# nitishsaDire/objectDetection_ssd

Hardware: AMD Instinct MI355X
Metric: images/sec SSD300-VGG16 train step (higher is better)
Workload: dtype f32 (tensors, accumulators, loss, SGD; the Winograd-domain products of the layers with >= 256 reduction channels are formed from three EXACT bf16 limbs per f32 operand on the bf16 MFMA -- six limb products per f32 product, dropped terms <= 2^-26 -- measured no further from f64 than the f32 MFMA; SSD

## Files before the change

### include/ssd_gfx950.h

```cpp
#ifndef SSD_GFX950_H
#define SSD_GFX950_H

#include <stddef.h>
#include <stdint.h>

#ifdef __cplusplus
extern "C" {
#endif

#define SSD_ABI_VERSION 1

enum ssd_status {
    SSD_OK = 0,
    SSD_ERR_BAD_SHAPE = -1,
    SSD_ERR_WORKSPACE = -2,
    SSD_ERR_NULL = -3,
    SSD_ERR_LAUNCH = -4,
    SSD_ERR_ALIGN = -5
};

int ssd_abi_version(void);
const char* ssd_status_string(int status);

typedef struct ssd_conv_geom {
// ... 100 lines not shown
int ssd_wino4_dy_transform(const float* dy, int ldy, const ssd_conv_geom* g, float* wgrad_planes, float* dgrad_planes_out,
                           float* bias_partial, void* stream);
size_t ssd_wino4_wgrad_gemm_workspace(const ssd_conv_geom* g, int ldy);
int ssd_wino4_wgrad_gemm(const float* wgrad_planes, const float* x_planes, int ldy, const float* bias_partial, float* dw_oihw, float* dbias,
                         const ssd_conv_geom* g, void* workspace, size_t workspace_bytes, void* stream);
int ssd_wino4_dy_transform_pooled(const float* dpool, const unsigned char* argmax, const float* y_pooled, int Hp, int Wp, int ldy,
                                  const ssd_conv_geom* g, float* wgrad_planes, float* dgrad_planes_out, float* bias_partial, void* stream);
int ssd_conv3x3_wino_wgrad_planes_pooled(const float* planes, const float* dpool, const unsigned char* argmax, const float* y_pooled,
                                         int Hp, int Wp, int ldy, float* dw_oihw, float* dbias, const ssd_conv_geom* g,
                                         float* dgrad_planes_out, void* workspace, size_t workspace_bytes, void* stream);
int ssd_conv3x3_wino_fwd_keep_bits(const float* x, const float* U_fwd, const float* bias, float* y, int ldy, const ssd_conv_geom* g, int relu,
                                   float* planes_keep, uint64_t* relu_bits_out, void* workspace, size_t workspace_bytes, void* stream);
int ssd_conv3x3_wino_fwd_pool_bits(const float* x, const float* U_fwd, const float* bias, float* y_pooled, uint8_t* argmax,
                                   const ssd_conv_geom* g, int ceil_mode, float* planes_keep, uint64_t* relu_bits_out, void* workspace,
                                   size_t workspace_bytes, void* stream);
int ssd_conv3x3_wino_dgrad_bits(const float* dy, int ldy, const float* U_bwd, int Co_pad, float* dx, const uint64_t* relu_bits, int accumulate,
                                const ssd_conv_geom* g, void* workspace, size_t workspace_bytes, void* stream);
int ssd_conv3x3_wino_dgrad_planes_bits(const float* dy_planes, const float* U_bwd, int Co_pad, float* dx, const uint64_t* relu_bits,
                                       int accumulate, const ssd_conv_geom* g, void* workspace, size_t workspace_bytes, void* stream);
int ssd_conv3x3_wino_wgrad_planes(const float* planes, const float* dy, int ldy, float* dw_oihw, float* dbias, const ssd_conv_geom* g,
                                  float* dgrad_planes_out, void* workspace, size_t workspace_bytes, void* stream);
int ssd_conv3x3_wino_dgrad_planes(const float* dy_planes, const float* U_bwd, int Co_pad, float* dx, const float* relu_mask,
                                  int accumulate, const ssd_conv_geom* g, void* workspace, size_t workspace_bytes, void* stream);
int ssd_conv1_first_wino_fwd(const float* x_nchw, const float* w_rows, const float* bias, float* planes, uint64_t* relu_bits, int N, int H, int W,
                             void* stream);
int ssd_conv3x3_wino_fwd_from_planes(const float* planes, const float* U_fwd, const float* bias, float* y, int ldy, float* y_pooled, uint8_t* argmax,
                                     const ssd_conv_geom* g, int relu, int ceil_mode, void* workspace, size_t workspace_bytes, void* stream);
int ssd_wino_weights_adj(const float* w_oihw, float* U_adj, int Co, int Ci, int Co_pad, void* stream);
size_t ssd_wino4_adj_planes_floats(const ssd_conv_geom* g);
int ssd_conv3x3_wino_dgrad_adj_gemm(const float* y_planes, int ldy, const float* U_adj, float* md_planes, const ssd_conv_geom* g, void* stream);
int ssd_wino4_adj_output(const float* md_planes, float* dx, const float* relu_mask, const uint64_t* relu_bits, int accumulate,
                         const ssd_conv_geom* g, void* stream);
int ssd_wino4_adj_output_to_planes(const float* md_planes, const float* relu_mask, const uint64_t* relu_bits, const ssd_conv_geom* g,
                                   const ssd_conv_geom* g_below, float* y_planes, float* bias_partial, void* stream);
int ssd_tune_set_wino_bias_tail(int on);
int ssd_tune_set_wino_xform_blocks(int blocks);
int ssd_tune_set_wino_fused(int mode);
int ssd_gemm_planes_x3v2(const void* a3, const void* w3, float* out, int M, int K, int N, int n_rows, int nbatch, int dither, void* stream);
int ssd_tune_set_x3_big(int mode);
int ssd_tune_set_x3_mfma(int rows);
int ssd_tune_set_gemm_nt(int mode);
int ssd_wino_uses_x3(int mo, int K);
int ssd_tune_set_wino_x3(int on);
size_t ssd_gemm_x3_weights_bytes(int rows, int K, int nbatch);
int ssd_gemm_x3_split_weights(const float* w, void* w3, int rows, int K, int nbatch, void* stream);
int ssd_gemm_planes_x3(const float* a, const void* w3, float* out, int M, int K, int N, int n_rows, int nbatch, void* stream);
// ... 158 lines not shown
```

### objectdetection_ssd_amd/Model.py

```python
from __future__ import annotations

import numbers
from typing import Dict, List, Optional

import torch
import torch.nn as nn

from . import ops
from .Util import ANCHORS_PER_CELL, ANCHORS_PER_CELL_512, subsampling

N_CLASSES = 21
MAX_FOREGROUND = 255
_VGG_CFG = (64, 64, "M", 128, 128, "M", 256, 256, 256, "M", 512, 512, 512, "M", 512, 512, 512, "M")


class _VGG16(nn.Module):

    def __init__(self):
        super().__init__()
        layers: List[nn.Module] = []
        cin = 3
        for v in _VGG_CFG:
            if v == "M":
                layers.append(nn.MaxPool2d(kernel_size=2, stride=2))
# ... 65 lines not shown
    for op in op_list:
        if op["op"] in ("conv", "conv_first"):
            names += [op["p"] + ".weight", op["p"] + ".bias"]
        elif op["op"] == "l2norm":
            names.append(op["p"])
        elif op["op"] == "head":
            names += [op["p"] + "_bb.weight", op["p"] + "_bb.bias", op["p"] + "_cl.weight", op["p"] + "_cl.bias"]
    return names


def _cat_flat(a: torch.Tensor, b: torch.Tensor) -> torch.Tensor:
    if (a.dim() == 1 and b.dim() == 1 and a.is_contiguous() and b.is_contiguous() and a.dtype == b.dtype
            and a.untyped_storage().data_ptr() == b.untyped_storage().data_ptr() and a.storage_offset() + a.numel() == b.storage_offset()):
        return torch.as_strided(a, (a.numel() + b.numel(),), (1,), a.storage_offset())
    return torch.cat((a, b))


class _Elided:

    dtype = torch.float32

    def __init__(self, shape):
        self.shape = tuple(shape)


class _SinkDict(dict):

    def __init__(self, sink):
        super().__init__()
        self._sink = sink
        self._held = None

    def __setitem__(self, name, tensor):
        super().__setitem__(name, tensor)
        if self._held is not None:
            self._held.append((name, tensor))
        else:
            self._sink(name, tensor)

    def hold(self):
        if self._held is None:
            self._held = []

    def release(self):
        held, self._held = self._held or [], None
        for name, tensor in held:
# ... 28 lines not shown
        self.pool_after: Dict[str, dict] = {}
        for op in self.ops:
            readers = [o for o in self.ops if o["x"] == op["y"]] if op["op"] == "conv" else []
            if (len(readers) == 1 and readers[0]["op"] == "pool" and (readers[0]["k"], readers[0]["s"], readers[0]["pad"]) == (2, 2, 0)
                    and op["relu"] and op["co"] % 4 == 0):
                self.pool_after[op["y"]] = readers[0]
        self._conv_of = {o["y"]: o for o in self.ops if o["op"] == "conv"}
        self.grad_sink = None
        self.grad_out = None
        self.sink_owns_grads = False
        self.sink_early = False
        self._test_side_delay = None
        self.grad_tap = None
        self.dual_dy = True
        self.keep_planes = True
        self.fuse_pool = True
        self.lazy_pool_grad = True
        self.first_fused = True
        self.wino_dilated = True
        self.relu_bits = True
        self.adjoint_dgrad = True
        self.first_wino = False
        self.adjoint_chain = True
        self.prof = None
        self.bf16 = False
        self.bf16_tensors = True
        self.x3 = False
        self.wino = True

    def _timed(self, label, tag, flops, fn):
        if self.prof is None:
            return fn()
        executed = flops
        if isinstance(flops, tuple):
            flops, executed = flops
        e0, e1 = torch.cuda.Event(enable_timing=True), torch.cuda.Event(enable_timing=True)
        e0.record()
        out = fn()
        e1.record()
        self.prof.append((label, tag, flops, e0, e1, executed))
        return out

    def schedule_key(self) -> tuple:
        return (self.bf16, self.bf16_tensors, self.x3, self.wino, self.WINO_TILE, self.WINO_MIN_CI, self.WINO_MIN_HW,
                self.WINO_WGRAD_MAX_HW, self.WINO_WGRAD_MIN_CI, self.X31_MIN_PIXELS, ops.wino_x3(4, 256), self.adjoint_dgrad,
                self.adjoint_chain, self.keep_planes, self.dual_dy, self.fuse_pool, self.lazy_pool_grad, self.relu_bits, self.wino_dilated,
                self.first_fused, self.first_wino, self.overlap_wgrad, self.batch_weights)

    def uses_weight_table(self) -> bool:
        return self.batch_weights and not self.x3 and (not self.bf16 or self.bf16_tensors)

    def _layouts(self, key: str, tensors, co_pad: int, need_bwd: bool):
        sig = tuple((t.data_ptr(), t._version) for t in tensors)
        ent = self._wcache.get(key)
        if ent is None or ent[0] != sig:
            w = tensors[0] if len(tensors) == 1 else torch.cat(list(tensors), 0)
            ent = [sig, w.detach().contiguous(), None, None]
            ent[2] = ops.weight_ohwi(ent[1], co_pad)
            self._wcache[key] = ent
        if need_bwd and ent[3] is None:
            ent[3] = ops.weight_ihwo(ent[1], co_pad)
        if self.x3 or (self.bf16 and not self.bf16_tensors):
            if len(ent) == 4:
                ent += [None, None]
            if ent[4] is None:
                ent[4] = ops.weight_split3(ent[2])
            if need_bwd and ent[5] is None:
                ent[5] = ops.weight_split3(ent[3])
            if self.x3:
                return ent[4], ent[5]
# ... 616 lines not shown
                                                         db_out=self._gout(name + ".bias")))
                        if side_ctx[0] is not None and defer:
                            deferred.append(wg)
                        else:
                            wg()
                        dw = None
                    if dw is not None:
                        grads[op["p"] + ".weight"], grads[op["p"] + ".bias"] = dw, db
                if self._wino_ok(g):
                    _, ub = self._wino_weights(op["p"], (P[op["p"] + ".weight"],), op["co"], adj=self._adj_ok(g))
                    if self._adj_ok(g):
                        raise RuntimeError(f"{op['p']}: its filter planes are laid out for the adjoint data gradient, which needs the forward's kept planes "
                                           "(the engine's keep_planes / dual_dy / adjoint_dgrad switches must not change between a forward and its backward)")
                    bits = aux.pop("bits:" + op["p"], None) if (dyp is not None or ops.wino_uses_full(g, 1) or isinstance(T[op["x"]], _Elided)) else None
                    def dgrad_rot(dx, acc, mask, dy=dy, ub=ub, g=g, dyp=dyp, bits=bits, name=op["p"]):
                        if isinstance(mask, _Elided):
                            if bits is None:
                                raise RuntimeError(f"{name}: its input was not stored and no ReLU bits were kept for its data gradient")
                            mask_t = None
                        else:
                            mask_t = mask
                        return ops.conv2d_dgrad_wino(None if isinstance(dy, ops.PooledGrad) else dy, ub, g, dx, mask_t, acc, planes=dyp,
                                                     bits=bits if mask is not None else None)
                    deliver(op["x"], lambda dx, acc, mask: self._timed("dgrad " + op["p"], "winograd_3x3", ops.wino_flops(g),
                                                                       lambda: dgrad_rot(dx, acc, mask)))
                    continue
                if self._x31_ok(g) and not to_bf16:
                    _, w3b = self._x31_weights(op["p"], (P[op["p"] + ".weight"],), op["co"])
                    deliver(op["x"], lambda dx, acc, mask: self._timed(
                        "dgrad " + op["p"], "gemm_planes_x3_kernel (1x1)", ops.conv_flops(g),
                        lambda: ops.conv1x1_dgrad_x3(dy, w3b, g, dx, mask, acc)))
                    continue
                _, wb = self._layouts(op["p"], (P[op["p"] + ".weight"],), op["co"], True)
                if to_bf16:
                    def boundary(dx, acc, mask, dy=dy, wb=wb, g=g, name=op["p"]):
                        if acc or mask is not None or dx is not None:
                            raise RuntimeError("the bf16 trunk's boundary tensor must have one consumer and no ReLU of its own")
                        d32 = self._timed("dgrad " + name, ops.igemm_tile(g, 1, self.bf16, self.x3) if self.prof is not None else "", ops.conv_flops(g),
                                          lambda: ops.conv2d_dgrad(dy, wb, g, None, None, False, bf16=self.bf16, w3=self._planes(name, True)))
                        return ops.cast_bf16(d32)
                    deliver(op["x"], boundary)
                    continue
                deliver(op["x"], lambda dx, acc, mask: self._timed(
                    "dgrad " + op["p"], ops.igemm_tile(g, 1, self.bf16, self.x3) if self.prof is not None else "", ops.conv_flops(g),
                    lambda: ops.conv2d_dgrad_x3(dy, wb, g, dx, mask, acc) if self.x3 else
                    ops.conv2d_dgrad(dy, wb, g, dx, mask, acc, bf16=self.bf16, w3=self._planes(op["p"], True))))
# ... 4 lines not shown
                yout = T[op["y"]]
                deliver(op["x"], lambda dx, acc, mask: (
                    ops.PooledGrad(dy, am, yout, xin.shape)
                    if (self.lazy_pool_grad and isinstance(xin, _Elided) and mask is not None and not acc and dx is None
                        and (op["k"], op["s"], op["pad"]) == (2, 2, 0)) else
                    ops.maxpool_bwd(dy, am, tuple(xin.shape), op["k"], op["s"], op["pad"], dx, y_gate=yout)
                    if (mask is not None and not acc) else
                    ops.maxpool_bwd(dy, am, tuple(xin.shape), op["k"], op["s"], op["pad"], dx, mask, acc)))
            elif kind == "l2norm":
                dy = G.pop(op["y"])
                xin = T[op["x"]]
                gamma = P[op["p"]].detach().reshape(-1)
                box = {}

                def run(dx, acc, mask, xin=xin, gamma=gamma, dy=dy, box=box):
                    if acc or mask is not None:
                        raise RuntimeError("L2-norm backward must deliver the first, non-final gradient of its input")
                    dx, box["dg"] = ops.l2norm_bwd(xin, gamma, dy, dg_out=self._gout(op["p"]))
                    return dx
                deliver(op["x"], run)
                grads[op["p"]] = box["dg"].reshape(P[op["p"]].shape)
            elif kind == "conv_first":
                dy = G.pop(op["y"])
                if need[op["p"] + ".weight"] or need[op["p"] + ".bias"]:
                    g = aux[op["y"]]
                    col = T["x_col"]
                    if col is None:
                        dw, db = self._timed("wgrad " + op["p"], "conv_first_wgrad_kernel", 2.0 * dy.numel() * 27,
                                             lambda: (ops.conv1_first_wgrad_bf16 if dy.dtype == torch.bfloat16 else ops.conv1_first_wgrad)(T["x"], dy, True))
                    else:
                        dw, db = self._timed("wgrad " + op["p"], ops.wgrad_tile(g, self.bf16) if self.prof is not None else "", 2.0 * dy.numel() * 27,
                                             lambda: ops.conv2d_wgrad(col, dy, g, g.Co, True))
                    grads[op["p"] + ".weight"], grads[op["p"] + ".bias"] = ops.first_weight_grad(dw), db
        if not joined:
            main.wait_event(join_event)
        if side_done is not None:
            main.wait_event(side_done)
        if wgrad_used:
            main.wait_event(self._wgrad_stream.record_event())
        if held:
            grads.release()
        return grads


class _SSD300Function(torch.autograd.Function):
    @staticmethod
# ... 171 lines not shown
```

### objectdetection_ssd_amd/_lib.py

```python
from __future__ import annotations

import ctypes as C
import os

PKG = os.path.dirname(os.path.abspath(__file__))
LIB_PATH = os.path.join(PKG, "libssd_gfx950.so")

SSD_ABI_VERSION = 1


class ConvGeom(C.Structure):
    _fields_ = [(n, C.c_int32) for n in ("N", "H", "W", "Ci", "Ho", "Wo", "Co", "R", "S", "stride", "pad", "dil")]


class ImageDesc(C.Structure):
    _fields_ = [("src_offset", C.c_int64)] + [(n, C.c_int32) for n in (
        "src_h", "src_w", "canvas_h", "canvas_w", "place_top", "place_left", "crop_top", "crop_left", "crop_h", "crop_w",
        "flip", "reserved")]


class WeightJob(C.Structure):
    _fields_ = [("w0", C.c_void_p), ("w1", C.c_void_p), ("out_fwd", C.c_void_p), ("out_bwd", C.c_void_p)] + [(n, C.c_int32) for n in (
        "co0", "co", "ci", "taps", "co_pad", "kind", "pad0", "pad1")]

# ... 96 lines not shown
    "ssd_conv3x3_wino_fwd": (_I, [_P, _P, _P, _P, _I, _G, _I, _I, _P, _Z, _P]),
    "ssd_conv3x3_wino_fwd_pool": (_I, [_P, _P, _P, _P, _P, _G, _I, _P, _P, _Z, _P]),
    "ssd_conv3x3_wino_fwd_keep": (_I, [_P, _P, _P, _P, _I, _G, _I, _P, _P, _Z, _P]),
    "ssd_weight_job_blocks": (_I, [_P]),
    "ssd_weights_prepare": (_I, [_P, _P, _I, _I, _P]),
    "ssd_wino4_bias_partial_floats": (_Z, [_G, _I]),
    "ssd_wino4_dy_transform": (_I, [_P, _I, _G, _P, _P, _P, _P]),
    "ssd_wino_weights_adj": (_I, [_P, _P, _I, _I, _I, _P]),
    "ssd_conv1_first_wino_fwd": (_I, [_P, _P, _P, _P, _P, _I, _I, _I, _P]),
    "ssd_conv3x3_wino_fwd_from_planes": (_I, [_P, _P, _P, _P, _I, _P, _P, _G, _I, _I, _P, _Z, _P]),
    "ssd_wino4_adj_planes_floats": (_Z, [_G]),
    "ssd_conv3x3_wino_dgrad_adj_gemm": (_I, [_P, _I, _P, _P, _G, _P]),
    "ssd_wino4_adj_output": (_I, [_P, _P, _P, _P, _I, _G, _P]),
    "ssd_wino4_adj_output_to_planes": (_I, [_P, _P, _P, _G, _G, _P, _P, _P]),
    "ssd_wino4_dy_transform_pooled": (_I, [_P, _P, _P, _I, _I, _I, _G, _P, _P, _P, _P]),
    "ssd_conv3x3_wino_wgrad_planes_pooled": (_I, [_P, _P, _P, _P, _I, _I, _I, _P, _P, _G, _P, _P, _Z, _P]),
    "ssd_wino4_wgrad_gemm_workspace": (_Z, [_G, _I]),
    "ssd_wino4_wgrad_gemm": (_I, [_P, _P, _I, _P, _P, _P, _G, _P, _Z, _P]),
    "ssd_conv3x3_wino_fwd_keep_bits": (_I, [_P, _P, _P, _P, _I, _G, _I, _P, _P, _P, _Z, _P]),
    "ssd_conv3x3_wino_fwd_pool_bits": (_I, [_P, _P, _P, _P, _P, _G, _I, _P, _P, _P, _Z, _P]),
    "ssd_conv3x3_wino_dgrad_planes_bits": (_I, [_P, _P, _I, _P, _P, _I, _G, _P, _Z, _P]),
    "ssd_conv3x3_wino_wgrad_planes": (_I, [_P, _P, _I, _P, _P, _G, _P, _P, _Z, _P]),
    "ssd_conv3x3_wino_dgrad_planes": (_I, [_P, _P, _I, _P, _P, _I, _G, _P, _Z, _P]),
    "ssd_conv3x3_wino_dgrad": (_I, [_P, _I, _P, _I, _P, _P, _I, _G, _I, _P, _Z, _P]),
    "ssd_conv3x3_wino_wgrad_workspace": (_Z, [_G, _I, _I]),
    "ssd_conv3x3_wino_wgrad": (_I, [_P, _P, _I, _P, _P, _G, _I, _P, _Z, _P]),
    "ssd_tune_set_wino_wgrad_tn": (_I, [_I]),
    "ssd_tune_set_wino_fused": (_I, [_I]),
    "ssd_tune_set_gemm_nt": (_I, [_I]),
    "ssd_tune_set_wino_bias_tail": (_I, [_I]),
    "ssd_tune_set_batched_units": (_I, [_I]),
    "ssd_tune_set_dgrad_parity": (_I, [_I]),
    "ssd_tune_set_wino_full": (_I, [_I]),
    "ssd_conv3x3_wino_uses_full": (_I, [_G, _I]),
    "ssd_conv3x3_wino_dgrad_bits": (_I, [_P, _I, _P, _I, _P, _P, _I, _G, _P, _Z, _P]),
    "ssd_tune_set_wino_xform_blocks": (_I, [_I]),
    "ssd_tune_set_wino_fused_stamps": (_I, [_P]),
    "ssd_tune_set_wino_fused_stagger": (_I, [_I]),
    "ssd_prof_gemm_begin": (_I, []),
    "ssd_prof_gemm_collect": (_I, [_P, _P, _I]),
    "ssd_prof_gemm_collect_kinds": (_I, [_P, _P, _P, _I]),
    "ssd_tune_set_igemm": (_I, [_I, _I]),
    "ssd_tune_set_igemm_lds_pad": (_I, [_I]),
    "ssd_tune_set_igemm_stamps": (_I, [_P]),
    "ssd_tune_set_wgrad": (_I, [_I, _I, _I]),
    "ssd_tune_set_wgrad_patch": (_I, [_I]),
# ... 57 lines not shown
```

### objectdetection_ssd_amd/csrc/wino_fused.hip

```cpp
#include "common.h"

namespace {

__device__ constexpr float F4_AT[4][6] = {{1, 1, 1, 1, 1, 0}, {0, 1, -1, 2, -2, 0}, {0, 1, 1, 4, 4, 0}, {0, 1, -1, 8, -8, 1}};

struct FusedParams {
    const float* V;
    const float* U;
    size_t plane_v, plane_u;
    int tiles, K, Nrows, Nout;
    int groups, nblk_n;
    float* out; int ldo; int Cvalid;
    const float* bias; const float* mask; const unsigned long long* mask_bits; int relu, accumulate;
    int H, W, TH, TW;
    float* yp; uint8_t* am; int Ho, Wo;
    unsigned long long* stamps;
    int stagger;
};

constexpr int FG = 32, FN = 64, FK = 64;
#ifndef WF_NS
#define WF_NS 5
#define WF_PD 3
#endif
constexpr int NS = WF_NS, PD = WF_PD;
constexpr int STAGE_F = (FG + FN) * FK;
constexpr int LOADS = 3;
constexpr int YS_F = FG * 16 * FN;
constexpr int LDS_F = NS * STAGE_F > YS_F ? NS * STAGE_F : YS_F;
static_assert(NS - PD >= 2, "a slot is re-filled no earlier than two barriers after its last read");
static_assert(LDS_F * 4 <= 160 * 1024, "LDS");

typedef __attribute__((address_space(3))) void lds_void;

template <int N> __device__ __forceinline__ void wait_vmcnt() { asm volatile("s_waitcnt vmcnt(%0)" ::"n"(N) : "memory"); }

template <int KCN>
__global__ __launch_bounds__(512, 2) void wino4_gemm_out_kernel(const FusedParams p) {
    __shared__ __attribute__((aligned(16))) float lds[LDS_F];
    const int tid = threadIdx.x, lane = tid & 63;
    const int wave = __builtin_amdgcn_readfirstlane(tid >> 6);
    const int mb = wave >> 2, nbw = wave & 3;
    const int nblk = p.groups * p.nblk_n;
    const int lid = xcd_swizzle(blockIdx.x, nblk);
    const int grp = lid / p.nblk_n, nb = lid - grp * p.nblk_n;
    const int tile0 = grp * FG, n0 = nb * FN;
    constexpr int S = 36 * KCN;
    const bool stamp = p.stamps != nullptr && (blockIdx.x & 15) == 0 && tid == 0;
    unsigned long long ts[8] = {0, 0, 0, 0, 0, 0, 0, 0};
    if (stamp) ts[0] = __builtin_readcyclecounter();
    if (p.stagger > 0 && blockIdx.x < 256) {
        const long long want = (long long)((blockIdx.x >> 3) & 7) * p.stagger;
        const long long t0 = (long long)__builtin_readcyclecounter();
        while ((long long)__builtin_readcyclecounter() - t0 < want) __builtin_amdgcn_s_sleep(64);
    }

    const int lrow = lane >> 4, pc = lane & 15;
    unsigned src_off[LOADS];
    bool is_a[LOADS];
    int lds_off[LOADS];
#pragma unroll
    for (int i = 0; i < LOADS; ++i) {
// ... 64 lines not shown
#endif
        __builtin_amdgcn_sched_barrier(0);
        mma4(c, cur, 1);
        mma4(c, cur, 2);
        __builtin_amdgcn_sched_barrier(0);
        if (s + 1 < S) {
            const int issued = (s + PD + 1 < S ? s + PD + 1 : S);
            const int ahead = issued - s - 2;
            if (ahead >= 3) wait_vmcnt<3 * LOADS>();
            else if (ahead == 2) wait_vmcnt<2 * LOADS>();
            else if (ahead == 1) wait_vmcnt<LOADS>();
            else wait_vmcnt<0>();
            __builtin_amdgcn_s_barrier();
            asm volatile("" ::: "memory");
            load_frags(nxt, (s + 1) % NS);
        }
        __builtin_amdgcn_sched_barrier(0);
        mma4(c, cur, 3);
    }

    if (stamp) ts[2] = __builtin_readcyclecounter();
    float* ys = lds;
    const int C4 = p.Nout >> 2;
    __builtin_amdgcn_s_barrier();
#pragma unroll
    for (int r = 0; r < 4; ++r) {
        float t[4][6];
#pragma unroll
        for (int b = 0; b < 6; ++b) {
            const float m0 = acc[b][r], m1 = acc[6 + b][r], m2 = acc[12 + b][r], m3 = acc[18 + b][r], m4 = acc[24 + b][r], m5 = acc[30 + b][r];
            const float s1 = m1 + m2, d1 = m1 - m2, s2 = m3 + m4, d2 = m3 - m4;
            t[0][b] = m0 + s1 + s2;
            t[1][b] = d1 + 2.f * d2;
            t[2][b] = s1 + 4.f * s2;
            t[3][b] = d1 + 8.f * d2 + m5;
        }
        float* dst = ys + (size_t)((mb * 16 + 4 * kq + r) * 16) * FN + nbw * 16 + r15;
#pragma unroll
        for (int i = 0; i < 4; ++i) {
            const float s1 = t[i][1] + t[i][2], d1 = t[i][1] - t[i][2], s2 = t[i][3] + t[i][4], d2 = t[i][3] - t[i][4];
            dst[(i * 4 + 0) * FN] = t[i][0] + s1 + s2;
            dst[(i * 4 + 1) * FN] = d1 + 2.f * d2;
            dst[(i * 4 + 2) * FN] = s1 + 4.f * s2;
            dst[(i * 4 + 3) * FN] = d1 + 8.f * d2 + t[i][5];
        }
    }
    asm volatile("s_waitcnt lgkmcnt(0)" ::: "memory");
    __builtin_amdgcn_s_barrier();
    if (stamp) ts[3] = __builtin_readcyclecounter();
    {
        const int tl = tid >> 4, c4l = tid & 15;
        const int tile = tile0 + tl, c4 = (n0 >> 2) + c4l;
        if (tile < p.tiles && c4 < C4) {
            const int tw = tile % p.TW, th = (tile / p.TW) % p.TH, n = tile / (p.TW * p.TH);
            const float* src = ys + (size_t)(tl * 16) * FN + c4l * 4;
            f32x4 bv = {0.f, 0.f, 0.f, 0.f};
            if (p.bias != nullptr) {
#pragma unroll
                for (int e = 0; e < 4; ++e) bv[e] = c4 * 4 + e < p.Cvalid ? p.bias[c4 * 4 + e] : 0.f;
            }
            if (p.yp == nullptr) {
                const unsigned long long word = p.mask_bits != nullptr ? p.mask_bits[(size_t)tile * C4 + c4] : 0ull;
#pragma unroll
                for (int a = 0; a < 4; ++a) {
                    const int oh = 4 * th + a;
                    if (oh >= p.H) continue;
#pragma unroll
                    for (int b = 0; b < 4; ++b) {
                        const int ow = 4 * tw + b;
                        if (ow >= p.W) continue;
                        f32x4 v = *reinterpret_cast<const f32x4*>(src + (a * 4 + b) * FN) + bv;
                        const size_t idx = (((size_t)n * p.H + oh) * p.W + ow) * p.ldo + c4 * 4;
                        if (p.accumulate) v += *reinterpret_cast<const f32x4*>(p.out + idx);
// ... 74 lines not shown
    return SSD_OK;
}
extern "C" int ssd_tune_set_wino_fused_stamps(uint64_t* device_buffer) {
    g_fused_stamps = reinterpret_cast<unsigned long long*>(device_buffer);
    return SSD_OK;
}

__attribute__((visibility("hidden"))) int ssd_internal_wino4_gemm_out(const float* V, const float* U, int tiles, int K, int Nrows, int Nout,
                                                                       float* out, int ldo, int Cvalid, const float* bias, const float* mask,
                                                                       const unsigned long long* mask_bits, int relu, int accumulate, int H, int W,
                                                                       int TH, int TW, float* yp, uint8_t* am, int Ho, int Wo, hipStream_t st) {
    if ((K != 64 && K != 128 && K != 256) || tiles <= 0 || Nout <= 0 || Nout % 4 != 0 || Nrows <= 0) return SSD_ERR_BAD_SHAPE;
    if ((size_t)tiles * K >= (1ull << 32) || (size_t)Nrows * K >= (1ull << 32)) return SSD_ERR_BAD_SHAPE;
    FusedParams p;
    p.V = V; p.U = U;
    p.plane_v = (size_t)tiles * K; p.plane_u = (size_t)Nrows * K;
    p.tiles = tiles; p.K = K; p.Nrows = Nrows; p.Nout = Nout;
    p.groups = ssd_cdiv(tiles, FG); p.nblk_n = ssd_cdiv(Nout, FN);
    p.out = out; p.ldo = ldo; p.Cvalid = Cvalid; p.bias = bias; p.mask = mask; p.mask_bits = mask_bits; p.relu = relu; p.accumulate = accumulate;
    p.H = H; p.W = W; p.TH = TH; p.TW = TW;
    p.yp = yp; p.am = am; p.Ho = Ho; p.Wo = Wo;
    p.stamps = g_fused_stamps;
    p.stagger = g_fused_stagger < 0 ? 0 : g_fused_stagger;
    const long long nblk = (long long)p.groups * p.nblk_n;
    if (nblk >= (1ll << 31)) return SSD_ERR_BAD_SHAPE;
    const int slot = ssd_internal_prof_open(2.0 * 36 * tiles * (double)K * (double)(p.nblk_n * FN), 1, st);
    switch (K / FK) {
        case 1: hipLaunchKernelGGL(wino4_gemm_out_kernel<1>, dim3((unsigned)nblk), dim3(512), 0, st, p); break;
        case 2: hipLaunchKernelGGL(wino4_gemm_out_kernel<2>, dim3((unsigned)nblk), dim3(512), 0, st, p); break;
        case 4: hipLaunchKernelGGL(wino4_gemm_out_kernel<4>, dim3((unsigned)nblk), dim3(512), 0, st, p); break;
        default: return SSD_ERR_BAD_SHAPE;
    }
    ssd_internal_prof_close(slot, st);
    SSD_CHECK_LAUNCH();
    return SSD_OK;
}

namespace {

__device__ constexpr float F4_BT[6][6] = {{4, 0, -5, 0, 1, 0}, {0, -4, -4, 1, 1, 0}, {0, 4, -4, -1, 1, 0},
                                          {0, -2, -1, 2, 1, 0}, {0, 2, -1, -2, 1, 0}, {0, 4, 0, -5, 0, 1}};

struct FullParams {
    const float* x;
    unsigned x_bytes;
    const float* U;
    size_t plane_u;
    int tiles, K, Nrows, Nout, groups, nblk_n;
    float* out; int ldo; int Cvalid;
    const float* bias; const float* mask; const unsigned long long* mask_bits; int relu, accumulate;
    int H, W, TH, TW;
    float* yp; uint8_t* am; int Ho, Wo;
    float* V_keep;
    unsigned long long* bits_out;
    unsigned long long* stamps;
};
// ... 290 lines not shown
```

### objectdetection_ssd_amd/csrc/winograd.hip

```cpp
#include <cstdlib>
#include "common.h"

int ssd_internal_gemm_batched(const float* a, const float* w, float* out, int M, int K, int N, int n_rows, int nbatch,
                              size_t batch_a_elems, size_t batch_w_elems, int ksplit, hipStream_t st);
int ssd_internal_gemm_batched_x3(const float* a, const void* w3, float* out, int M, int K, int N, int n_rows, int nbatch, size_t batch_a_elems,
                                 hipStream_t st);
int ssd_internal_gemm_tn_x3(const float* a, const float* c, float* out, int M, int N, int K, int lda, int ldc, int nbatch, int ksplit,
                            int ksteps_per_split, size_t batch_a, size_t batch_c, hipStream_t st);
int ssd_internal_wino4_gemm_out(const float* V, const float* U, int tiles, int K, int Nrows, int Nout, float* out, int ldo, int Cvalid,
                                const float* bias, const float* mask, const unsigned long long* mask_bits, int relu, int accumulate, int H,
                                int W, int TH, int TW, float* yp, uint8_t* am, int Ho, int Wo, hipStream_t st);

int ssd_internal_wino4_full(const float* x, const float* U, int tiles, int K, int Nrows, int Nout, float* out, int ldo, int Cvalid,
                            const float* bias, const float* mask, const unsigned long long* mask_bits, int relu, int accumulate, int H, int W,
                            int TH, int TW, float* yp, uint8_t* am, int Ho, int Wo, float* V_keep, unsigned long long* bits_out, hipStream_t st);

namespace {

struct Lat { int D; int h0[4], w0[4]; };
__device__ __forceinline__ void lat_tile(const int (&first)[4], int D, int t, int& off, int& base) {
    off = 0;
#pragma unroll
    for (int a = 1; a < 4; ++a)
        if (a < D && t >= first[a]) off = a;
    base = 4 * (t - first[off]);
}

__global__ void wino_weight_kernel(const float* __restrict__ w, float* __restrict__ U, int Co, int Ci, int Nrows, int K, int mode) {
    const size_t total = (size_t)Nrows * K;
    for (size_t i = (size_t)blockIdx.x * blockDim.x + threadIdx.x; i < total; i += (size_t)gridDim.x * blockDim.x) {
        const int k = (int)(i % K), n = (int)(i / K);
        const int co = mode == 0 ? n : k, ci = mode == 0 ? k : n;
        float g[3][3];
#pragma unroll
// ... 1373 lines not shown
    return wino_conv(4, dy, Co_pad, U_bwd, g->Ci, dx, g->Ci, g->Ci, nullptr, nullptr, 0, accumulate, g->N, g->H, g->W, workspace, workspace_bytes,
                     (hipStream_t)stream, nullptr, nullptr, nullptr, nullptr, reinterpret_cast<const unsigned long long*>(relu_bits), g->dil);
}
extern "C" int ssd_conv3x3_wino_dgrad_planes_bits(const float* dy_planes, const float* U_bwd, int Co_pad, float* dx, const uint64_t* relu_bits,
                                                  int accumulate, const ssd_conv_geom* g, void* workspace, size_t workspace_bytes,
                                                  void* stream) {
    if (!dy_planes || !U_bwd || !dx || !workspace || !relu_bits) return SSD_ERR_NULL;
    if (!wino_geom_ok(g) || Co_pad % 32 != 0 || Co_pad < g->Co || g->Ci % 4 != 0) return SSD_ERR_BAD_SHAPE;
    if (!ssd_aligned16(dy_planes) || !ssd_aligned16(dx) || !ssd_aligned16(workspace) || !ssd_aligned16(U_bwd) || ((uintptr_t)relu_bits & 7))
        return SSD_ERR_ALIGN;
    return wino_conv(4, nullptr, Co_pad, U_bwd, g->Ci, dx, g->Ci, g->Ci, nullptr, nullptr, 0, accumulate, g->N, g->H, g->W, workspace,
                     workspace_bytes, (hipStream_t)stream, nullptr, nullptr, dy_planes, nullptr,
                     reinterpret_cast<const unsigned long long*>(relu_bits), g->dil);
}
extern "C" int ssd_conv3x3_wino_dgrad_planes(const float* dy_planes, const float* U_bwd, int Co_pad, float* dx, const float* relu_mask,
                                             int accumulate, const ssd_conv_geom* g, void* workspace, size_t workspace_bytes, void* stream) {
    if (!dy_planes || !U_bwd || !dx || !workspace) return SSD_ERR_NULL;
    if (!wino_geom_ok(g) || Co_pad % 32 != 0 || Co_pad < g->Co || g->Ci % 4 != 0) return SSD_ERR_BAD_SHAPE;
    if (!ssd_aligned16(dy_planes) || !ssd_aligned16(dx) || !ssd_aligned16(workspace) || !ssd_aligned16(U_bwd) ||
        (relu_mask && !ssd_aligned16(relu_mask)))
        return SSD_ERR_ALIGN;
    return wino_conv(4, nullptr, Co_pad, U_bwd, g->Ci, dx, g->Ci, g->Ci, nullptr, relu_mask, 0, accumulate, g->N, g->H, g->W, workspace,
                     workspace_bytes, (hipStream_t)stream, nullptr, nullptr, dy_planes, nullptr, nullptr, g->dil);
}
namespace {
int wino_wgrad(const float* x, const float* planes, const float* dy, int ldy, float* dw_oihw, float* dbias, const ssd_conv_geom* g, int mo,
               float* dgrad_planes, void* workspace, size_t workspace_bytes, void* stream, const PoolSrc* pool) {
    if (!dy || !dw_oihw || !workspace) return SSD_ERR_NULL;
    if (!wino_geom_ok(g) || g->Ci % 4 != 0 || ldy % 4 != 0 || ldy < g->Co || (mo != 2 && mo != 4)) return SSD_ERR_BAD_SHAPE;
    if (!ssd_aligned16(dy) || !ssd_aligned16(workspace) || !ssd_aligned16(dw_oihw)) return SSD_ERR_ALIGN;
    const WinoWgradPlan w = wino_wgrad_plan(g, ldy, mo);
    if (w.tiles >= (1ull << 31)) return SSD_ERR_BAD_SHAPE;
    if (workspace_bytes < w.yb + w.vb + w.zb + w.pb) return SSD_ERR_WORKSPACE;
    hipStream_t st = (hipStream_t)stream;
    char* base = static_cast<char*>(workspace);
    float* Yt = reinterpret_cast<float*>(base);
    float* Vt = reinterpret_cast<float*>(base + w.yb);
    float* Zs = reinterpret_cast<float*>(base + w.yb + w.vb);
    float* part = reinterpret_cast<float*>(base + w.yb + w.vb + w.zb);
    const int gy = (w.Tpad / 32) * ((ldy / 4 + 7) / 8), gx = (w.Tpad / 32) * ((g->Ci / 4 + 7) / 8);
    const dim3 gyd(gy > 16384 ? 16384 : gy), gxd(gx > 16384 ? 16384 : gx);
    int dy_bias_blocks = 0;
    if (dgrad_planes != nullptr && !(mo == 4 && (g_wgrad_tn || planes != nullptr))) return SSD_ERR_BAD_SHAPE;
    if (g->dil != 1 && (pool != nullptr || !(mo == 4 && (g_wgrad_tn || planes != nullptr)))) return SSD_ERR_BAD_SHAPE;
    if (mo == 4 && (g_wgrad_tn || planes != nullptr)) {
        const int c4 = ldy / 4;
// ... 424 lines not shown
```

### objectdetection_ssd_amd/ops.py

```python
from __future__ import annotations

import contextlib
import ctypes as C
from typing import List, Optional, Tuple

import torch

from . import _lib
from ._lib import ConvGeom, check


def _stream() -> int:
    return torch.cuda.current_stream().cuda_stream


_current_device = torch.cuda.current_device


def _req(t: torch.Tensor, name: str, dtype=torch.float32) -> torch.Tensor:
    if not isinstance(t, torch.Tensor):
        raise TypeError(f"{name}: expected a tensor")
    if not t.is_cuda:
        raise RuntimeError(f"{name}: the gfx950 path needs a device tensor (got {t.device}); there is no CPU fallback")
    if t.device.index != _current_device():
# ... 1281 lines not shown
        _req(relu_mask, "relu_mask")
    lib = _lib.load()
    ws = workspace(lib.ssd_conv3x3_wino_workspace(C.byref(g), 1, mo), dev, "wino")
    if bits is not None:
        _req(bits, "bits", torch.int64)
        if mo != 4 or tuple(bits.shape) != (wino_planes_shape(g)[1], g.Ci // 4) or g.Ci % 4 != 0:
            raise ValueError("conv2d_dgrad_wino: bits need F(4x4) filters and one word per (tile, channel quad)")
        if planes is None:
            check(lib.ssd_conv3x3_wino_dgrad_bits(dy.data_ptr(), co_pad, u_bwd.data_ptr(), co_pad, dx.data_ptr(), bits.data_ptr(), int(accumulate),
                                                  C.byref(g), ws.data_ptr(), ws.numel(), _stream()), "conv2d_dgrad_wino")
            return dx
        check(lib.ssd_conv3x3_wino_dgrad_planes_bits(planes.data_ptr(), u_bwd.data_ptr(), co_pad, dx.data_ptr(), bits.data_ptr(), int(accumulate),
                                                     C.byref(g), ws.data_ptr(), ws.numel(), _stream()), "conv2d_dgrad_wino")
        return dx
    if planes is not None:
        check(lib.ssd_conv3x3_wino_dgrad_planes(planes.data_ptr(), u_bwd.data_ptr(), co_pad, dx.data_ptr(), _ptr(relu_mask), int(accumulate),
                                                C.byref(g), ws.data_ptr(), ws.numel(), _stream()), "conv2d_dgrad_wino")
        return dx
    check(lib.ssd_conv3x3_wino_dgrad(dy.data_ptr(), co_pad, u_bwd.data_ptr(), co_pad, dx.data_ptr(), _ptr(relu_mask), int(accumulate),
                                     C.byref(g), mo, ws.data_ptr(), ws.numel(), _stream()), "conv2d_dgrad_wino")
    return dx


def conv2d_wgrad_wino(x: Optional[torch.Tensor], dy: torch.Tensor, g: ConvGeom, ldy: int, want_bias: bool = True, mo: int = 2,
                      planes: Optional[torch.Tensor] = None, dgrad_planes: bool = False,
                      dw_out: Optional[torch.Tensor] = None, db_out: Optional[torch.Tensor] = None):
    pooled = isinstance(dy, PooledGrad)
    if pooled and planes is None:
        raise ValueError("conv2d_wgrad_wino: a pooled gradient needs the kept forward planes")
    if not pooled:
        _req(dy, "dy")
    if planes is not None:
        _req(planes, "planes")
        if mo != 4 or tuple(planes.shape) != tuple(wino_planes_shape(g)):
            raise ValueError("conv2d_wgrad_wino: planes do not match the geometry")
    else:
        _req(x, "x")
        if tuple(x.shape) != (g.N, g.H, g.W, g.Ci):
            raise ValueError("conv2d_wgrad_wino: shapes do not match the geometry")
    if not pooled and dy.numel() != g.N * g.H * g.W * ldy:
        raise ValueError("conv2d_wgrad_wino: shapes do not match the geometry")
    lib = _lib.load()
    nbytes = lib.ssd_conv3x3_wino_wgrad_workspace(C.byref(g), ldy, mo)
    if nbytes == 0:
        raise ValueError("conv2d_wgrad_wino: not a 3x3 / stride 1 / pad 1 geometry")
    dev = planes.device if pooled else dy.device
# ... 185 lines not shown
```

Measured before the change: 1652.

## Fold first-conv weight gradient into conv1_2 Winograd data-gradient epilogue

In the backward pass, the data gradient of conv1_2 (Ci=64) is no longer written to memory and then re-read by a separate conv1_1 weight-gradient pass. The fused Winograd GEMM kernel's epilogue now masks the gradient with the ReLU bits, loads the matching 6x6x3 input patch into LDS, and forms per-block partial dW/db products with an f32 MFMA. A two-stage reduction over blocks then produces dW and db. This removes a full-resolution gradient write and read plus the im2col wgrad pass, at the cost of extra LDS use, which may lower occupancy, and two small reduction kernels.

```diff
diff --git a/include/ssd_gfx950.h b/include/ssd_gfx950.h
--- a/include/ssd_gfx950.h
+++ b/include/ssd_gfx950.h
@@ -146,6 +146,10 @@
                                   float* dgrad_planes_out, void* workspace, size_t workspace_bytes, void* stream);
 int ssd_conv3x3_wino_dgrad_planes(const float* dy_planes, const float* U_bwd, int Co_pad, float* dx, const float* relu_mask,
                                   int accumulate, const ssd_conv_geom* g, void* workspace, size_t workspace_bytes, void* stream);
+size_t ssd_conv3x3_wino_dgrad_first_wgrad_workspace(const ssd_conv_geom* g);
+int ssd_conv3x3_wino_dgrad_planes_first_wgrad(const float* dy_planes, const float* U_bwd, int Co_pad, const uint64_t* relu_bits,
+                                              const float* relu_mask, int accumulate, const ssd_conv_geom* g, const float* x_nchw,
+                                              float* dw_oihw, float* dbias, void* workspace, size_t workspace_bytes, void* stream);
 int ssd_conv1_first_wino_fwd(const float* x_nchw, const float* w_rows, const float* bias, float* planes, uint64_t* relu_bits, int N, int H, int W,
                              void* stream);
 int ssd_conv3x3_wino_fwd_from_planes(const float* planes, const float* U_fwd, const float* bias, float* y, int ldy, float* y_pooled, uint8_t* argmax,
diff --git a/objectdetection_ssd_amd/Model.py b/objectdetection_ssd_amd/Model.py
--- a/objectdetection_ssd_amd/Model.py
+++ b/objectdetection_ssd_amd/Model.py
@@ -111,6 +111,11 @@
 
     def __init__(self, shape):
         self.shape = tuple(shape)
+
+
+class _Folded:
+    """Stands in the gradient table for an activation gradient that was consumed where it was formed (`first_wgrad_fold`): the
+    producer of that activation has nothing left to do in the backward."""
 
 
 class _SinkDict(dict):
@@ -185,6 +190,8 @@
         self.adjoint_dgrad = True
         self.first_wino = False
         self.adjoint_chain = True
+        self.first_wgrad_fold = True
+        self._first_of = {o["y"]: o for o in self.ops if o["op"] == "conv_first"}
         self.prof = None
         self.bf16 = False
         self.bf16_tensors = True
@@ -208,7 +215,7 @@
         return (self.bf16, self.bf16_tensors, self.x3, self.wino, self.WINO_TILE, self.WINO_MIN_CI, self.WINO_MIN_HW,
                 self.WINO_WGRAD_MAX_HW, self.WINO_WGRAD_MIN_CI, self.X31_MIN_PIXELS, ops.wino_x3(4, 256), self.adjoint_dgrad,
                 self.adjoint_chain, self.keep_planes, self.dual_dy, self.fuse_pool, self.lazy_pool_grad, self.relu_bits, self.wino_dilated,
-                self.first_fused, self.first_wino, self.overlap_wgrad, self.batch_weights)
+                self.first_fused, self.first_wino, self.overlap_wgrad, self.batch_weights, self.first_wgrad_fold)
 
     def uses_weight_table(self) -> bool:
         return self.batch_weights and not self.x3 and (not self.bf16 or self.bf16_tensors)
@@ -871,6 +878,19 @@
                             mask_t = mask
                         return ops.conv2d_dgrad_wino(None if isinstance(dy, ops.PooledGrad) else dy, ub, g, dx, mask_t, acc, planes=dyp,
                                                      bits=bits if mask is not None else None)
+                    first = self._first_of.get(op["x"]) if self.first_wgrad_fold else None
+                    if (first is not None and self.consumers[op["x"]] == 1 and dyp is not None and not self.bf16 and not self.x3
+                            and (need[first["p"] + ".weight"] or need[first["p"] + ".bias"]) and T["x"].dtype == torch.float32
+                            and (bits is not None or torch.is_tensor(T[op["x"]])) and ops.wino_first_wgrad_ok(g)):
+                        def dgrad_first(dx, acc, mask, ub=ub, g=g, dyp=dyp, bits=bits, name=first["p"]):
+                            dw1, db1 = ops.conv2d_dgrad_wino_first_wgrad(dyp, ub, g, T["x"], bits=bits, relu_mask=None if bits is not None else mask,
+                                                                         accumulate=acc, dw_out=self._gout(name + ".weight"),
+                                                                         db_out=self._gout(name + ".bias"))
+                            grads[name + ".weight"], grads[name + ".bias"] = dw1, db1
+                            return _Folded()
+                        deliver(op["x"], lambda dx, acc, mask: self._timed("dgrad " + op["p"] + " + wgrad " + first["p"], "winograd_3x3",
+                                                                           ops.wino_flops(g), lambda: dgrad_first(dx, acc, mask)))
+                        continue
                     deliver(op["x"], lambda dx, acc, mask: self._timed("dgrad " + op["p"], "winograd_3x3", ops.wino_flops(g),
                                                                        lambda: dgrad_rot(dx, acc, mask)))
                     continue
@@ -921,6 +941,8 @@
                 grads[op["p"]] = box["dg"].reshape(P[op["p"]].shape)
             elif kind == "conv_first":
                 dy = G.pop(op["y"])
+                if isinstance(dy, _Folded):
+                    continue
                 if need[op["p"] + ".weight"] or need[op["p"] + ".bias"]:
                     g = aux[op["y"]]
                     col = T["x_col"]
diff --git a/objectdetection_ssd_amd/_lib.py b/objectdetection_ssd_amd/_lib.py
--- a/objectdetection_ssd_amd/_lib.py
+++ b/objectdetection_ssd_amd/_lib.py
@@ -142,6 +142,8 @@
     "ssd_conv3x3_wino_dgrad_planes_bits": (_I, [_P, _P, _I, _P, _P, _I, _G, _P, _Z, _P]),
     "ssd_conv3x3_wino_wgrad_planes": (_I, [_P, _P, _I, _P, _P, _G, _P, _P, _Z, _P]),
     "ssd_conv3x3_wino_dgrad_planes": (_I, [_P, _P, _I, _P, _P, _I, _G, _P, _Z, _P]),
+    "ssd_conv3x3_wino_dgrad_first_wgrad_workspace": (_Z, [_G]),
+    "ssd_conv3x3_wino_dgrad_planes_first_wgrad": (_I, [_P, _P, _I, _P, _P, _I, _G, _P, _P, _P, _P, _Z, _P]),
     "ssd_conv3x3_wino_dgrad": (_I, [_P, _I, _P, _I, _P, _P, _I, _G, _I, _P, _Z, _P]),
     "ssd_conv3x3_wino_wgrad_workspace": (_Z, [_G, _I, _I]),
     "ssd_conv3x3_wino_wgrad": (_I, [_P, _P, _I, _P, _P, _G, _I, _P, _Z, _P]),
diff --git a/objectdetection_ssd_amd/csrc/wino_fused.hip b/objectdetection_ssd_amd/csrc/wino_fused.hip
--- a/objectdetection_ssd_amd/csrc/wino_fused.hip
+++ b/objectdetection_ssd_amd/csrc/wino_fused.hip
@@ -16,6 +16,7 @@
     float* yp; uint8_t* am; int Ho, Wo;
     unsigned long long* stamps;
     int stagger;
+    const float* x0; float* part;
 };
 
 constexpr int FG = 32, FN = 64, FK = 64;
@@ -28,16 +29,18 @@
 constexpr int LOADS = 3;
 constexpr int YS_F = FG * 16 * FN;
 constexpr int LDS_F = NS * STAGE_F > YS_F ? NS * STAGE_F : YS_F;
+constexpr int XP_F = 3 * 6 * 6;
+constexpr int XS_F = FG * XP_F;
 static_assert(NS - PD >= 2, "a slot is re-filled no earlier than two barriers after its last read");
-static_assert(LDS_F * 4 <= 160 * 1024, "LDS");
+static_assert((LDS_F + XS_F) * 4 <= 160 * 1024, "LDS");
 
 typedef __attribute__((address_space(3))) void lds_void;
 
 template <int N> __device__ __forceinline__ void wait_vmcnt() { asm volatile("s_waitcnt vmcnt(%0)" ::"n"(N) : "memory"); }
 
-template <int KCN>
+template <int KCN, bool FW = false>
 __global__ __launch_bounds__(512, 2) void wino4_gemm_out_kernel(const FusedParams p) {
-    __shared__ __attribute__((aligned(16))) float lds[LDS_F];
+    __shared__ __attribute__((aligned(16))) float lds[FW ? LDS_F + XS_F : LDS_F];
     const int tid = threadIdx.x, lane = tid & 63;
     const int wave = __builtin_amdgcn_readfirstlane(tid >> 6);
     const int mb = wave >> 2, nbw = wave & 3;
@@ -148,6 +151,24 @@
     if (stamp) ts[2] = __builtin_readcyclecounter();
     float* ys = lds;
     const int C4 = p.Nout >> 2;
+    constexpr int XPT = (XP_F + 15) / 16;
+    [[maybe_unused]] float xv[XPT];
+    [[maybe_unused]] int f_tw = 0, f_th = 0, f_n = 0;
+    [[maybe_unused]] bool f_valid = false;
+    if constexpr (FW) {
+        const int tile = tile0 + (tid >> 4);
+        f_valid = tile < p.tiles;
+        f_tw = tile % p.TW; f_th = (tile / p.TW) % p.TH; f_n = tile / (p.TW * p.TH);
+#pragma unroll
+        for (int u = 0; u < XPT; ++u) {
+            const int j = (tid & 15) + 16 * u;
+            const int c = j / 36, rr = (j % 36) / 6, cc = j % 6;
+            const int ih = 4 * f_th - 1 + rr, iw = 4 * f_tw - 1 + cc;
+            xv[u] = 0.f;
+            if (f_valid && j < XP_F && (unsigned)ih < (unsigned)p.H && (unsigned)iw < (unsigned)p.W)
+                xv[u] = p.x0[(((size_t)f_n * 3 + c) * p.H + ih) * p.W + iw];
+        }
+    }
     __builtin_amdgcn_s_barrier();
 #pragma unroll
     for (int r = 0; r < 4; ++r) {
@@ -171,10 +192,84 @@
             dst[(i * 4 + 3) * FN] = d1 + 8.f * d2 + t[i][5];
         }
     }
+    if constexpr (FW) {
+        float* xs = lds + LDS_F;
+#pragma unroll
+        for (int u = 0; u < XPT; ++u) {
+            const int j = (tid & 15) + 16 * u;
+            if (j < XP_F) xs[(tid >> 4) * XP_F + j] = xv[u];
+        }
+    }
     asm volatile("s_waitcnt lgkmcnt(0)" ::: "memory");
     __builtin_amdgcn_s_barrier();
     if (stamp) ts[3] = __builtin_readcyclecounter();
-    {
+    if constexpr (FW) {
+        {
+            const int tl = tid >> 4, c4l = tid & 15;
+            float* img = ys + (size_t)(tl * 16) * FN + c4l * 4;
+            const unsigned long long word = (f_valid && p.mask_bits != nullptr) ? p.mask_bits[(size_t)(tile0 + tl) * 16 + c4l] : 0ull;
+#pragma unroll
+            for (int a = 0; a < 4; ++a) {
+#pragma unroll
+                for (int b = 0; b < 4; ++b) {
+                    const int oh = 4 * f_th + a, ow = 4 * f_tw + b;
+                    const bool ok = f_valid && oh < p.H && ow < p.W;
+                    f32x4 v = *reinterpret_cast<const f32x4*>(img + (a * 4 + b) * FN);
+                    if (p.mask_bits != nullptr) {
+#pragma unroll
+                        for (int e = 0; e < 4; ++e) v[e] = (ok && ((word >> ((a * 4 + b) * 4 + e)) & 1ull)) ? v[e] : 0.f;
+                    } else if (p.mask != nullptr) {
+                        f32x4 mk = {0.f, 0.f, 0.f, 0.f};
+                        if (ok) mk = *reinterpret_cast<const f32x4*>(p.mask + (((size_t)f_n * p.H + oh) * p.W + ow) * FN + c4l * 4);
+#pragma unroll
+                        for (int e = 0; e < 4; ++e) v[e] = mk[e] > 0.f ? v[e] : 0.f;
+                    } else {
+#pragma unroll
+                        for (int e = 0; e < 4; ++e) v[e] = ok ? v[e] : 0.f;
+                    }
+                    *reinterpret_cast<f32x4*>(img + (a * 4 + b) * FN) = v;
+                }
+            }
+        }
+        __syncthreads();
+        const float* xs = lds + LDS_F;
+        const int lr = lane & 31, lh = lane >> 5;
+        const int tap_c = lr % 3, tap_rs = lr / 3;
+        const int tap_off = lr < 27 ? tap_c * 36 + (tap_rs / 3) * 6 + tap_rs % 3 : 0;
+        const float b_const = lr == 27 ? 1.f : 0.f;
+        f32x16 pacc[2];
+#pragma unroll
+        for (int i = 0; i < 2; ++i)
+#pragma unroll
+            for (int r = 0; r < 16; ++r) pacc[i][r] = 0.f;
+#pragma unroll
+        for (int tt = 0; tt < 4; ++tt) {
+            const int tl = 4 * wave + tt;
+            const float* yt = ys + (size_t)(tl * 16) * FN + lr;
+            const float* xt = xs + tl * XP_F + tap_off;
+#pragma unroll
+            for (int q = 0; q < 8; ++q) {
+                const int px = 2 * q + lh;
+                const float bv = lr < 27 ? xt[(px >> 2) * 6 + (px & 3)] : b_const;
+#pragma unroll
+                for (int i = 0; i < 2; ++i) pacc[i] = __builtin_amdgcn_mfma_f32_32x32x2f32(yt[px * FN + 32 * i], bv, pacc[i], 0, 0, 0);
+            }
+        }
+        __syncthreads();
+#pragma unroll
+        for (int i = 0; i < 2; ++i)
+#pragma unroll
+            for (int r = 0; r < 16; ++r) lds[wave * 2048 + (32 * i + (r & 3) + 8 * (r >> 2) + 4 * lh) * 32 + lr] = pacc[i][r];
+        __syncthreads();
+#pragma unroll
+        for (int e = 0; e < 4; ++e) {
+            const int idx = e * 512 + tid;
+            float v = lds[idx];
+#pragma unroll
+            for (int w = 1; w < 8; ++w) v += lds[w * 2048 + idx];
+            p.part[(size_t)grp * 2048 + idx] = v;
+        }
+    } else {
         const int tl = tid >> 4, c4l = tid & 15;
         const int tile = tile0 + tl, c4 = (n0 >> 2) + c4l;
         if (tile < p.tiles && c4 < C4) {
@@ -295,6 +390,7 @@
     p.yp = yp; p.am = am; p.Ho = Ho; p.Wo = Wo;
     p.stamps = g_fused_stamps;
     p.stagger = g_fused_stagger < 0 ? 0 : g_fused_stagger;
+    p.x0 = nullptr; p.part = nullptr;
     const long long nblk = (long long)p.groups * p.nblk_n;
     if (nblk >= (1ll << 31)) return SSD_ERR_BAD_SHAPE;
     const int slot = ssd_internal_prof_open(2.0 * 36 * tiles * (double)K * (double)(p.nblk_n * FN), 1, st);
@@ -305,6 +401,76 @@
         default: return SSD_ERR_BAD_SHAPE;
     }
     ssd_internal_prof_close(slot, st);
+    SSD_CHECK_LAUNCH();
+    return SSD_OK;
+}
+
+namespace {
+constexpr int FWR_BLOCKS = 128;
+constexpr int FWR_CHUNK = 64;
+__global__ __launch_bounds__(256) void first_wgrad_presum_kernel(const float* __restrict__ part, float* __restrict__ part2, int groups) {
+    const int idx = blockIdx.x * 256 + threadIdx.x;
+    const int g0 = blockIdx.y * FWR_CHUNK, g1 = min(g0 + FWR_CHUNK, groups);
+    float s[4] = {0.f, 0.f, 0.f, 0.f};
+    for (int b = g0; b < g1; b += 4) {
+#pragma unroll
+        for (int u = 0; u < 4; ++u)
+            if (b + u < g1) s[u] += part[(size_t)(b + u) * 2048 + idx];
+    }
+    part2[(size_t)blockIdx.y * 2048 + idx] = (s[0] + s[1]) + (s[2] + s[3]);
+}
+__global__ __launch_bounds__(256) void first_wgrad_reduce_kernel(const float* __restrict__ part, float* __restrict__ dw, float* __restrict__ db,
+                                                                 int groups) {
+    __shared__ float red[16][17];
+    const int e = threadIdx.x & 15, sl = threadIdx.x >> 4;
+    const int idx = blockIdx.x * 16 + e;
+    float s[4] = {0.f, 0.f, 0.f, 0.f};
+    for (int b = sl; b < groups; b += 64) {
+#pragma unroll
+        for (int u = 0; u < 4; ++u)
+            if (b + 16 * u < groups) s[u] += part[(size_t)(b + 16 * u) * 2048 + idx];
+    }
+    red[sl][e] = (s[0] + s[1]) + (s[2] + s[3]);
+    __syncthreads();
+    if (sl == 0) {
+        float v = red[0][e];
+        for (int k = 1; k < 16; ++k) v += red[k][e];
+        const int k = idx & 31, co = idx >> 5;
+        if (k < 27 && dw != nullptr) dw[co * 27 + (k % 3) * 9 + k / 3] = v;
+        if (k == 27 && db != nullptr) db[co] = v;
+    }
+}
+}
+
+__attribute__((visibility("hidden"))) size_t ssd_internal_wino4_first_wgrad_part_floats(size_t tiles) {
+    const size_t groups = (tiles + FG - 1) / FG;
+    return (groups + (groups + FWR_CHUNK - 1) / FWR_CHUNK) * 2048;
+}
+__attribute__((visibility("hidden"))) int ssd_internal_wino4_gemm_first_wgrad(const float* V, const float* U, int tiles, int Nrows, const float* mask,
+                                                                               const unsigned long long* mask_bits, int H, int W, int TH, int TW,
+                                                                               const float* x_nchw, float* part, float* dw_oihw, float* dbias,
+                                                                               hipStream_t st) {
+    if (tiles <= 0 || Nrows <= 0 || (size_t)tiles * 64 >= (1ull << 32)) return SSD_ERR_BAD_SHAPE;
+    FusedParams p;
+    p.V = V; p.U = U;
+    p.plane_v = (size_t)tiles * 64; p.plane_u = (size_t)Nrows * 64;
+    p.tiles = tiles; p.K = 64; p.Nrows = Nrows; p.Nout = 64;
+    p.groups = ssd_cdiv(tiles, FG); p.nblk_n = 1;
+    p.out = nullptr; p.ldo = 64; p.Cvalid = 64; p.bias = nullptr; p.mask = mask; p.mask_bits = mask_bits; p.relu = 0; p.accumulate = 0;
+    p.H = H; p.W = W; p.TH = TH; p.TW = TW;
+    p.yp = nullptr; p.am = nullptr; p.Ho = 0; p.Wo = 0;
+    p.stamps = g_fused_stamps;
+    p.stagger = g_fused_stagger < 0 ? 0 : g_fused_stagger;
+    p.x0 = x_nchw; p.part = part;
+    const int slot = ssd_internal_prof_open(2.0 * 36 * tiles * 64.0 * 64.0, 1, st);
+    hipLaunchKernelGGL((wino4_gemm_out_kernel<1, true>), dim3((unsigned)p.groups), dim3(512), 0, st, p);
+    ssd_internal_prof_close(slot, st);
+    SSD_CHECK_LAUNCH();
+    const int chunks = ssd_cdiv(p.groups, FWR_CHUNK);
+    float* part2 = part + (size_t)p.groups * 2048;
+    hipLaunchKernelGGL(first_wgrad_presum_kernel, dim3(8, chunks), dim3(256), 0, st, part, part2, p.groups);
+    SSD_CHECK_LAUNCH();
+    hipLaunchKernelGGL(first_wgrad_reduce_kernel, dim3(FWR_BLOCKS), dim3(256), 0, st, part2, dw_oihw, dbias, chunks);
     SSD_CHECK_LAUNCH();
     return SSD_OK;
 }
diff --git a/objectdetection_ssd_amd/csrc/winograd.hip b/objectdetection_ssd_amd/csrc/winograd.hip
--- a/objectdetection_ssd_amd/csrc/winograd.hip
+++ b/objectdetection_ssd_amd/csrc/winograd.hip
@@ -10,6 +10,9 @@
 int ssd_internal_wino4_gemm_out(const float* V, const float* U, int tiles, int K, int Nrows, int Nout, float* out, int ldo, int Cvalid,
                                 const float* bias, const float* mask, const unsigned long long* mask_bits, int relu, int accumulate, int H,
                                 int W, int TH, int TW, float* yp, uint8_t* am, int Ho, int Wo, hipStream_t st);
+size_t ssd_internal_wino4_first_wgrad_part_floats(size_t tiles);
+int ssd_internal_wino4_gemm_first_wgrad(const float* V, const float* U, int tiles, int Nrows, const float* mask, const unsigned long long* mask_bits,
+                                        int H, int W, int TH, int TW, const float* x_nchw, float* part, float* dw_oihw, float* dbias, hipStream_t st);
 
 int ssd_internal_wino4_full(const float* x, const float* U, int tiles, int K, int Nrows, int Nout, float* out, int ldo, int Cvalid,
                             const float* bias, const float* mask, const unsigned long long* mask_bits, int relu, int accumulate, int H, int W,
@@ -1429,6 +1432,30 @@
         return SSD_ERR_ALIGN;
     return wino_conv(4, nullptr, Co_pad, U_bwd, g->Ci, dx, g->Ci, g->Ci, nullptr, relu_mask, 0, accumulate, g->N, g->H, g->W, workspace,
                      workspace_bytes, (hipStream_t)stream, nullptr, nullptr, dy_planes, nullptr, nullptr, g->dil);
+}
+namespace {
+bool first_wgrad_ok(const ssd_conv_geom* g, int Co_pad) {
+    return wino_geom_ok(g) && g->dil == 1 && g->Ci == 64 && Co_pad == 64 && g->Co <= 64 && use_fused(4, 64, 64) &&
+           (size_t)g->N * ((g->H + 3) / 4) * ((g->W + 3) / 4) < (1ull << 25);
+}
+}
+extern "C" size_t ssd_conv3x3_wino_dgrad_first_wgrad_workspace(const ssd_conv_geom* g) {
+    if (!first_wgrad_ok(g, 64)) return 0;
+    return align256(ssd_internal_wino4_first_wgrad_part_floats((size_t)g->N * ((g->H + 3) / 4) * ((g->W + 3) / 4)) * sizeof(float));
+}
+extern "C" int ssd_conv3x3_wino_dgrad_planes_first_wgrad(const float* dy_planes, const float* U_bwd, int Co_pad, const uint64_t* relu_bits,
+                                                         const float* relu_mask, int accumulate, const ssd_conv_geom* g, const float* x_nchw,
+                                                         float* dw_oihw, float* dbias, void* workspace, size_t workspace_bytes, void* stream) {
+    if (!dy_planes || !U_bwd || !x_nchw || !workspace || (!dw_oihw && !dbias)) return SSD_ERR_NULL;
+    if (!first_wgrad_ok(g, Co_pad) || accumulate != 0) return SSD_ERR_BAD_SHAPE;
+    if (!ssd_aligned16(dy_planes) || !ssd_aligned16(U_bwd) || !ssd_aligned16(workspace) || (relu_mask && !ssd_aligned16(relu_mask)) ||
+        ((uintptr_t)relu_bits & 7))
+        return SSD_ERR_ALIGN;
+    if (workspace_bytes < ssd_conv3x3_wino_dgrad_first_wgrad_workspace(g)) return SSD_ERR_WORKSPACE;
+    const int TH = (g->H + 3) / 4, TW = (g->W + 3) / 4;
+    return ssd_internal_wino4_gemm_first_wgrad(dy_planes, U_bwd, g->N * TH * TW, g->Ci, relu_mask,
+                                               reinterpret_cast<const unsigned long long*>(relu_bits), g->H, g->W, TH, TW, x_nchw,
+                                               static_cast<float*>(workspace), dw_oihw, dbias, (hipStream_t)stream);
 }
 namespace {
 int wino_wgrad(const float* x, const float* planes, const float* dy, int ldy, float* dw_oihw, float* dbias, const ssd_conv_geom* g, int mo,
diff --git a/objectdetection_ssd_amd/ops.py b/objectdetection_ssd_amd/ops.py
--- a/objectdetection_ssd_amd/ops.py
+++ b/objectdetection_ssd_amd/ops.py
@@ -1327,6 +1327,44 @@
     return dx
 
 
+def wino_first_wgrad_ok(g: ConvGeom) -> bool:
+    return _lib.load().ssd_conv3x3_wino_dgrad_first_wgrad_workspace(C.byref(g)) != 0
+
+
+def conv2d_dgrad_wino_first_wgrad(planes: torch.Tensor, u_bwd: torch.Tensor, g: ConvGeom, x_nchw: torch.Tensor,
+                                  bits: Optional[torch.Tensor] = None, relu_mask: Optional[torch.Tensor] = None, accumulate: bool = False,
+                                  want_bias: bool = True, dw_out: Optional[torch.Tensor] = None, db_out: Optional[torch.Tensor] = None):
+    mo = _wino_mo(u_bwd)
+    co_pad = _wino_filter(u_bwd, "u_bwd", g.Ci, None)
+    _req(planes, "planes"); _req(x_nchw, "x")
+    if accumulate:
+        raise ValueError("conv2d_dgrad_wino_first_wgrad: no dx is written, so there is none to accumulate into")
+    if mo != 4 or tuple(planes.shape) != (36, wino_planes_shape(g)[1], co_pad):
+        raise ValueError("conv2d_dgrad_wino_first_wgrad: planes do not match the geometry")
+    if tuple(x_nchw.shape) != (g.N, 3, g.H, g.W):
+        raise ValueError("conv2d_dgrad_wino_first_wgrad: x (N,3,H,W) of the layer's geometry")
+    if bits is not None:
+        _req(bits, "bits", torch.int64)
+        if tuple(bits.shape) != (wino_planes_shape(g)[1], g.Ci // 4) or g.Ci % 4 != 0:
+            raise ValueError("conv2d_dgrad_wino_first_wgrad: bits need one word per (tile, channel quad)")
+    elif relu_mask is not None:
+        _req(relu_mask, "relu_mask")
+        if tuple(relu_mask.shape) != (g.N, g.H, g.W, g.Ci):
+            raise ValueError("conv2d_dgrad_wino_first_wgrad: relu_mask (N,H,W,Ci)")
+    lib = _lib.load()
+    nbytes = lib.ssd_conv3x3_wino_dgrad_first_wgrad_workspace(C.byref(g))
+    if nbytes == 0:
+        raise ValueError("conv2d_dgrad_wino_first_wgrad: not a geometry of the fused K = 64 data gradient (Ci = Co_pad = 64, dilation 1)")
+    dev = planes.device
+    ws = workspace(nbytes, dev, "first_wgrad")
+    dw = _grad_dst(dw_out, (64, 3, 3, 3), dev, "dw_out")
+    db = _grad_dst(db_out, (64,), dev, "db_out") if want_bias else None
+    check(lib.ssd_conv3x3_wino_dgrad_planes_first_wgrad(planes.data_ptr(), u_bwd.data_ptr(), co_pad, _ptr(bits), _ptr(None if bits is not None else relu_mask),
+                                                        0, C.byref(g), x_nchw.data_ptr(), dw.data_ptr(), _ptr(db), ws.data_ptr(), ws.numel(),
+                                                        _stream()), "conv2d_dgrad_wino_first_wgrad")
+    return dw, db
+
+
 def conv2d_wgrad_wino(x: Optional[torch.Tensor], dy: torch.Tensor, g: ConvGeom, ldy: int, want_bias: bool = True, mo: int = 2,
                       planes: Optional[torch.Tensor] = None, dgrad_planes: bool = False,
                       dw_out: Optional[torch.Tensor] = None, db_out: Optional[torch.Tensor] = None):
```

Result: no change. 1661, median of 6 (+0.5%).
